# TheJacksonLaboratory/cnn_autoencoder

Measured on AMD Instinct MI355X. Metric: tiles/sec, compress+decompress round trip of 1024x1024x3 histology tiles, higher is better.
Workload: dtype f32 (f16x3 split MFMA: 3 f16 MFMAs per product, fp32 accumulate)

## Files before the change

### cnn_autoencoder_amd/_lib.py

```python
from __future__ import annotations

import ctypes
import os
import subprocess
import threading

import torch

_HERE = os.path.dirname(os.path.abspath(__file__))
LIB_PATH = os.environ.get('CAE_LIB') or os.path.join(_HERE, 'libcae_hip.so')
_lock = threading.Lock()
_lib = None

c_void_p = ctypes.c_void_p
c_int = ctypes.c_int
c_size_t = ctypes.c_size_t
c_float = ctypes.c_float

SYMBOLS = {
    'cae_version': (c_int, []),
    'cae_last_error': (ctypes.c_char_p, []),
    'cae_free': (None, [c_void_p]),
    'cae_model_create': (c_int, [c_int, c_int, c_int, c_int, c_int, ctypes.POINTER(c_void_p)]),
    'cae_model_destroy': (None, [c_void_p]),
    'cae_model_set_layer': (c_int, [c_void_p, c_int, c_int, c_int, c_int, c_void_p, c_void_p, c_void_p, c_void_p]),
    'cae_model_set_layer_act': (c_int, [c_void_p, c_int, c_int, c_int, c_void_p, c_void_p]),
    'cae_model_set_precision': (c_int, [c_void_p, c_int]),
    'cae_last_range_ticket': (ctypes.c_int64, []),
    'cae_range_check': (c_int, [c_void_p, ctypes.c_int64, c_void_p]),
    'cae_thread_force_fp32': (None, [c_int]),
    'cae_model_effective_precision': (c_int, [c_void_p, c_void_p]),
    'cae_model_set_entropy': (c_int, [c_void_p, c_int, c_int, c_void_p, c_void_p, c_void_p, c_void_p]),
    'cae_analysis': (c_int, [c_void_p, c_void_p, c_int, c_int, c_int, c_int, c_void_p, c_void_p]),
    'cae_analysis_levels': (c_int, [c_void_p, c_void_p, c_int, c_int, c_int, c_int, c_void_p, c_void_p, c_void_p]),
    'cae_synthesis': (c_int, [c_void_p, c_void_p, c_int, c_int, c_int, c_void_p, c_int, c_void_p, c_void_p]),
    'cae_model_set_layer_stage': (c_int, [c_void_p, c_int, c_int, c_int, c_void_p, c_void_p, c_void_p, c_void_p, c_int,
                                           c_int, c_int]),
    'cae_model_set_color_layer': (c_int, [c_void_p, c_int, c_int, c_int, c_void_p, c_void_p]),
    'cae_synthesis_multiscale': (c_int, [c_void_p, c_void_p, c_int, c_int, c_int, c_void_p, c_int, c_void_p, c_void_p,
                                          c_void_p]),
    'cae_analysis_symbols': (c_int, [c_void_p, c_void_p, c_int, c_int, c_int, c_int, c_void_p, c_void_p]),
    'cae_synthesis_symbols': (c_int, [c_void_p, c_void_p, c_int, c_int, c_int, c_void_p, c_int, c_void_p]),
    'cae_synthesis_scale': (c_int, [c_void_p, c_void_p, c_int, c_int, c_int, c_int, c_void_p, c_int, c_void_p]),
    'cae_synthesis_symbols_scale': (c_int, [c_void_p, c_void_p, c_int, c_int, c_int, c_int, c_void_p, c_int, c_void_p]),
    'cae_gdn_forward': (c_int, [c_void_p, c_int, c_int, c_void_p, c_int, c_int, c_int, c_void_p, c_void_p]),
    'cae_quantize': (c_int, [c_void_p, c_void_p, c_int, c_int, c_void_p, c_void_p]),
    'cae_quantize_export': (c_int, [c_void_p, c_void_p, c_int, c_int, c_void_p, c_int, c_void_p]),
    'cae_copy_to_host': (c_int, [c_void_p, c_void_p, c_size_t]),
    'cae_dequantize': (c_int, [c_void_p, c_void_p, c_int, c_int, c_void_p, c_void_p]),
    'cae_model_set_density': (c_int, [c_void_p, c_int, c_int, c_void_p, c_void_p, c_void_p, c_void_p, c_float]),
    'cae_model_set_likelihood_form': (c_int, [c_void_p, c_int]),
    'cae_likelihood': (c_int, [c_void_p, c_void_p, c_int, c_int, c_void_p, c_void_p, c_void_p, c_void_p]),
    'cae_tile_ssim': (c_int, [c_void_p, c_void_p, c_int, c_int, c_int, c_int, c_void_p, c_void_p, c_size_t, c_void_p]),
    'cae_tile_delta_e': (c_int, [c_void_p, c_void_p, c_int, c_size_t, c_void_p, c_void_p, c_size_t, c_void_p]),
    'cae_u8hwc_to_planes': (c_int, [c_void_p, c_int, c_int, c_int, c_int, c_void_p, c_void_p]),
    'cae_avgpool2': (c_int, [c_void_p, c_int, c_int, c_int, c_void_p, c_void_p]),
    'cae_msssim_level': (c_int, [c_void_p, c_void_p, c_int, c_int, c_int, c_void_p, c_void_p, c_void_p, c_size_t, c_void_p]),
    'cae_tile_sse': (c_int, [c_void_p, c_void_p, c_int, c_size_t, c_void_p, c_void_p]),
    'cae_model_set_profiling': (c_int, [c_void_p, c_int]),
    'cae_model_get_profile': (c_int, [c_void_p, c_int, c_void_p, c_int, c_void_p, c_int]),
    'cae_t_packed_bytes': (c_size_t, [c_int, c_int, c_int]),
    'cae_t_pack_weights': (c_int, [c_void_p, c_int, c_int, c_int, c_int, c_void_p, c_void_p]),
    'cae_t_from_nchw': (c_int, [c_void_p, c_int, c_int, c_int, c_int, c_int, c_void_p, c_void_p, c_void_p]),
    'cae_t_to_nchw': (c_int, [c_void_p, c_int, c_int, c_int, c_int, c_int, c_void_p, c_void_p]),
    'cae_t_set_samples_per_block': (c_int, [c_int]),
# ... 220 lines not shown
```

### cnn_autoencoder_amd/csrc/cae_api.hip

```cpp
#include "cae_hip.h"
#include "cae_internal.hpp"
#include "cae_kernels.hpp"
#include "cae_kernels_f16.hpp"
#include "cae_launch.hpp"
#include "cae_pack.hpp"

#include <algorithm>
#include <cmath>
#include <cstdio>
#include <cstdlib>
#include <cstring>
#include <string>

namespace cae {

thread_local std::string g_last_error;
thread_local int64_t g_last_ticket = 0;
thread_local int g_force_fp32 = 0;

int fail(int code, const char *fmt, ...) {
    char buf[512];
    va_list ap;
    va_start(ap, fmt);
    vsnprintf(buf, sizeof buf, fmt, ap);
// ... 5 lines not shown
void dev_free(void *p) { (void)hipFree(p); }

int DevBuf::alloc(size_t n) {
    reset();
    HIP_TRY(hipMalloc(&p, n));
    bytes = n;
    return CAE_OK;
}

int DevBuf::upload(const void *src, size_t n) {
    CAE_TRY(alloc(n));
    HIP_TRY(hipMemcpy(p, src, n, hipMemcpyHostToDevice));
    return CAE_OK;
}

int Model::ensure_ws(int which, size_t bytes) {
    DevBuf &b = ws[which];
    if (b.bytes >= bytes) return CAE_OK;
    if (b) {
        HIP_TRY(hipDeviceSynchronize());
        b.reset();
    }
    return b.alloc((bytes + (1u << 20)) & ~(size_t)((1u << 20) - 1));
}

int Model::order_stream(void *stream) {
    if (last_stream_set && last_stream != stream) {
        if (!order_event) HIP_TRY(hipEventCreateWithFlags((hipEvent_t *)&order_event, hipEventDisableTiming));
        HIP_TRY(hipEventRecord((hipEvent_t)order_event, (hipStream_t)last_stream));
        HIP_TRY(hipStreamWaitEvent((hipStream_t)stream, (hipEvent_t)order_event, 0));
    }
    last_stream = stream;
    last_stream_set = true;
    return CAE_OK;
}

int Model::ensure_device() {
    if (!zero) {
        CAE_TRY(zero.alloc(1024));
        HIP_TRY(hipMemset(zero.p, 0, 1024));
    }
    if (medians_dirty && ent.channels > 0) {
        CAE_TRY(medians_dev.upload(ent.medians));
        medians_dirty = false;
    }
    if (density_dirty && !density.empty()) {
// ... 570 lines not shown
            if ((rc = launch_conv(m->ks, l.ct, l.gdn, l.cin, a, st))) return rc;
        }
        prof.end();
        if (!last && levels && levels[i]) {
            const size_t t2 = (size_t)n * l.cout * a.OH * a.OW;
            if (f16)
                hipLaunchKernelGGL(c8s_to_nchw_kernel<false>, dim3(ew_grid(t2)), dim3(256), 0, st, (const char *)a.out,
                                   levels[i], n, l.cout, a.OH, a.OW, l.ct * 4);
            else
                hipLaunchKernelGGL(c8_to_nchw_kernel, dim3(ew_grid(t2)), dim3(256), 0, st, (const float *)a.out,
                                   levels[i], n, l.cout, a.OH * a.OW, l.ct * 4);
            HIP_TRY(hipGetLastError());
        }
        cur = (const float *)a.out;
        cur_planes = l.ct * 4;
        ch = a.OH;
        cw = a.OW;
        cur_idx = out_idx;
    }
    return CAE_OK;
}

static int synthesis_impl(cae_model_t *mm, const float *latents, const int32_t *symbols, int n, int lh, int lw, void *out,
                          int fmt, float *const *bridges, float *const *colors, void *stream, int scale = 0);

int cae_synthesis(cae_model_t *mm, const float *latents, int n, int lh, int lw, void *out, int fmt,
                  float *const *bridges, void *stream) {
    if (!latents) return fail(CAE_ERR_ARG, "NULL argument");
    return synthesis_impl(mm, latents, nullptr, n, lh, lw, out, fmt, bridges, nullptr, stream);
}

int cae_synthesis_multiscale(cae_model_t *mm, const float *latents, int n, int lh, int lw, void *out, int fmt,
                             float *const *bridges, float *const *colors, void *stream) {
    if (!latents) return fail(CAE_ERR_ARG, "NULL argument");
    return synthesis_impl(mm, latents, nullptr, n, lh, lw, out, fmt, bridges, colors, stream);
}

int cae_synthesis_symbols(cae_model_t *mm, const int32_t *symbols, int n, int lh, int lw, void *out, int fmt,
                          void *stream) {
    if (!symbols) return fail(CAE_ERR_ARG, "NULL argument");
    return synthesis_impl(mm, nullptr, symbols, n, lh, lw, out, fmt, nullptr, nullptr, stream);
}

static int check_scale(cae_model_t *mm, int scale) {
    Model *m = reinterpret_cast<Model *>(mm);
    if (!m) return fail(CAE_ERR_ARG, "NULL argument");
    if (scale < 0 || scale >= m->L) return fail(CAE_ERR_ARG, "scale %d outside 0..%d", scale, m->L - 1);
    return CAE_OK;
}

int cae_synthesis_scale(cae_model_t *mm, const float *latents, int n, int lh, int lw, int scale, void *out, int fmt,
                        void *stream) {
    if (!latents) return fail(CAE_ERR_ARG, "NULL argument");
    CAE_TRY(check_scale(mm, scale));
    return synthesis_impl(mm, latents, nullptr, n, lh, lw, out, fmt, nullptr, nullptr, stream, scale);
}

int cae_synthesis_symbols_scale(cae_model_t *mm, const int32_t *symbols, int n, int lh, int lw, int scale, void *out,
                                int fmt, void *stream) {
    if (!symbols) return fail(CAE_ERR_ARG, "NULL argument");
    CAE_TRY(check_scale(mm, scale));
    return synthesis_impl(mm, nullptr, symbols, n, lh, lw, out, fmt, nullptr, nullptr, stream, scale);
}

static int synthesis_impl(cae_model_t *mm, const float *latents, const int32_t *symbols, int n, int lh, int lw, void *out,
                          int fmt, float *const *bridges, float *const *colors, void *stream, int scale) {
    Model *m = reinterpret_cast<Model *>(mm);
    if (!m || !out) return fail(CAE_ERR_ARG, "NULL argument");
    const int stop = m->L - 1 - scale, nrun = stop + 1;
    if (symbols && m->ent.channels == 0) return fail(CAE_ERR_ARG, "entropy model not set");
    if (n < 1 || lh < 1 || lw < 1) return fail(CAE_ERR_ARG, "bad latent batch %dx%dx%d", n, lh, lw);
    if (fmt != CAE_FMT_U8_HWC && fmt != CAE_FMT_F32_NCHW) return fail(CAE_ERR_ARG, "bad pixel format %d", fmt);
    for (auto &l : m->dec)
        if (!l.set) return fail(CAE_ERR_ARG, "synthesis layer not set");
    for (int i = 0; colors && i + 1 < m->L; ++i)
        if (colors[i] && ((lh << (i + 1)) <= m->ks / 2 || (lw << (i + 1)) <= m->ks / 2))
            return fail(CAE_ERR_ARG, "colour layer %d input %d x %d too small for reflect padding %d", i, lh << (i + 1),
                        lw << (i + 1), m->ks / 2);
    if (scale > 0) {
        const Layer &l = m->dec[stop];
        if (!l.color_wp) return fail(CAE_ERR_ARG, "colour layer %d not set", stop);
        if ((lh << nrun) <= m->ks / 2 || (lw << nrun) <= m->ks / 2)
            return fail(CAE_ERR_ARG, "colour layer %d input %d x %d too small for reflect padding %d", stop, lh << nrun,
                        lw << nrun, m->ks / 2);
    }
    hipStream_t st = (hipStream_t)stream;
    std::lock_guard<std::mutex> lk(m->mu);
    int rc;
    if ((rc = m->ensure_device()) || (rc = m->order_stream(stream))) return rc;
// ... 28 lines not shown
    if (maxact && ((rc = m->ensure_ws(1, maxact)) || (rc = m->ensure_ws(2, maxact)))) return rc;
    if (maxact && need_third_slot && (rc = m->ensure_ws(3, maxact))) return rc;

    ProfScope prof(m, CAE_SYNTHESIS, st);
    prof.begin();
    const size_t tot = (size_t)n * p0 * lh * lw;
    if (f16)
        hipLaunchKernelGGL(nchw_to_c8s_kernel<true>, dim3(ew_grid(tot)), dim3(256), 0, st, latents, (char *)m->ws[0].p, n,
                           m->c_bn, lh, lw, p0, flag, symbols, m->medians_dev.get<float>());
    else
        hipLaunchKernelGGL(nchw_to_c8_kernel, dim3(ew_grid(tot)), dim3(256), 0, st, latents, (float *)m->ws[0].p, n,
                           m->c_bn, lh * lw, p0, symbols, m->medians_dev.get<float>());
    HIP_TRY(hipGetLastError());
    prof.end();

    bool use_pmap = false;
    if (f16 && scale == 0 && m->L >= 2 && m->ks == 3 && getenv("CAE_NO_PMAP") == nullptr) {
        const Layer &lp = m->dec[m->L - 2], &ll = m->dec[m->L - 1];
        use_pmap = ll.wp_pmap16 && !ll.gdn && ll.stages.empty() && lp.stages.empty() && lp.ct <= 4 && lp.cout == ll.cin &&
                   !(bridges && bridges[m->L - 2]) && !(colors && colors[m->L - 2]);
    }
    if (use_pmap) maxact = std::max(maxact, (size_t)n * (lh << (m->L - 1)) * (lw << (m->L - 1)) * 128);
    if (use_pmap && ((rc = m->ensure_ws(1, maxact)) || (rc = m->ensure_ws(2, maxact)))) return rc;

    const float *cur = (const float *)m->ws[0].p;
    int cur_planes = p0, ch = lh, cw = lw;
    int cur_idx = 0;
    for (int i = 0; i < nrun; ++i) {
        const Layer &l = m->dec[i];
        const bool last = i == m->L - 1;
        if (use_pmap && last) {
            prof.begin();
            const int gtx = (cw + 15) / 16, gty = (ch + 15) / 16;
            hipLaunchKernelGGL(pmap_gather_kernel, dim3((unsigned)((size_t)n * gtx * gty)), dim3(256), 0, st, cur,
                               l.bias.get<float>(), out, n, ch, cw, l.cout, fmt == CAE_FMT_U8_HWC ? OUT_U8HWC : OUT_NCHW, gtx,
                               gty);
            HIP_TRY(hipGetLastError());
            prof.end();
            break;
        }
        if (!l.stages.empty() && (rc = run_stages(m, l, true, n, ch, cw, cur, cur_idx, cur_planes, st, f16, flag))) return rc;
        const int out_idx = pick_slot(cur_idx, cur_idx);
        LayerArgs a = layer_args(m, cur, cur_planes, last ? out : m->ws[out_idx].p, n, ch, cw, 2 * ch, 2 * cw, l.ct, l.cout,
                                 last ? (fmt == CAE_FMT_U8_HWC ? OUT_U8HWC : OUT_NCHW) : OUT_C8, l.act, flag);
        a.wp = l.wp.get<float>();
        a.bias = l.bias.get<float>();
        a.gp = l.gp.get<float>();
        a.beta = l.beta.get<float>();
        if (use_pmap && i == m->L - 2) {
            a.outfmt = OUT_PMAP;
            a.pm = m->dec[m->L - 1].wp_pmap16.p;
        }
        prof.begin();
        if (f16) {
            a.gp = l.gp16.get<float>();
            if (last && l.wp_edge16 && last_f16_fits(m->ks, l.cin)) {
                a.wp = l.wp_edge16.get<float>();
                if ((rc = launch_last_f16(m->ks, l.cin, a, st))) return rc;
            } else {
                if (l.act && l.ct > 4)
// ... 26 lines not shown
            HIP_TRY(hipGetLastError());
        }
        cur = (const float *)a.out;
        cur_planes = l.ct * 4;
        ch = a.OH;
        cw = a.OW;
        cur_idx = out_idx;
    }
    if (scale > 0) {
        const Layer &l = m->dec[stop];
        const int ofmt = fmt == CAE_FMT_U8_HWC ? OUT_U8HWC : OUT_NCHW;
        prof.begin();
        if (l.color_w4) {
            if ((rc = launch_color_small(m->ks, f16, cur, cur_planes, l.cout, l.color_w4.get<float>(),
                                         l.color_bias.get<float>(), n, ch, cw, l.color_cout, out, ofmt, flag, st)))
                return rc;
        } else {
            float *img = ofmt == OUT_NCHW ? (float *)out : (float *)m->ws[pick_slot(cur_idx, cur_idx)].p;
            if ((rc = launch_color(m, l, f16, cur, cur_planes, n, ch, cw, img, flag, st))) return rc;
            if (ofmt == OUT_U8HWC && (rc = launch_nchw_to_u8hwc(img, out, n, l.color_cout, (size_t)ch * cw, st))) return rc;
        }
        prof.end();
    }
    return CAE_OK;
}

int cae_gdn_forward(cae_model_t *mm, int track, int index, const float *x, int n, int h, int w, float *y, void *stream) {
    Model *m = reinterpret_cast<Model *>(mm);
    if (!m || !x || !y) return fail(CAE_ERR_ARG, "NULL argument");
    Layer *lp;
    CAE_TRY(layer_of(m, track, index, lp));
    if (n < 1 || h < 1 || w < 1) return fail(CAE_ERR_ARG, "bad tensor shape");
    hipStream_t st = (hipStream_t)stream;
    std::lock_guard<std::mutex> lk(m->mu);
    const Layer &l = *lp;
    if (!l.set || !l.gdn) return fail(CAE_ERR_ARG, "layer has no GDN");
    const int planes = l.ct * 4;
    int rc;
    if ((rc = m->ensure_device()) || (rc = m->order_stream(stream))) return rc;
    if ((rc = m->ensure_ws(0, (size_t)n * planes * h * w * 32))) return rc;
    const size_t tot = (size_t)n * planes * h * w;
    hipLaunchKernelGGL(nchw_to_c8_kernel, dim3(ew_grid(tot)), dim3(256), 0, st, x, (float *)m->ws[0].p, n, l.cout, h * w,
                       planes);
    HIP_TRY(hipGetLastError());
    LayerArgs a = layer_args(m, (const float *)m->ws[0].p, planes, y, n, h, w, h, w, l.ct, l.cout, OUT_NCHW, 0, nullptr);
    a.gp = l.gp.get<float>();
// ... 285 lines not shown
```

### cnn_autoencoder_amd/csrc/cae_internal.hpp

```cpp
#pragma once
#include <cstdarg>
#include <cstddef>
#include <cstdint>
#include <mutex>
#include <utility>
#include <vector>

namespace cae {

int fail(int code, const char *fmt, ...);

void dev_free(void *p);

struct DevBuf {
    void *p = nullptr;
    size_t bytes = 0;
    DevBuf() = default;
    DevBuf(DevBuf &&o) noexcept : p(o.p), bytes(o.bytes) {
        o.p = nullptr;
        o.bytes = 0;
    }
    DevBuf &operator=(DevBuf &&o) noexcept {
        if (this != &o) {
            reset();
// ... 80 lines not shown
    DevBuf buf;
    uint64_t version = 0;
    size_t enc = 0, cdf = 0, lut = 0, len = 0, off = 0;
};

struct Model {
    int c_org = 0, c_net = 0, c_bn = 0, L = 0, ks = 3;
    std::vector<Layer> enc, dec;
    EntropyTables ent;
    uint64_t ent_version = 0;
    DevEntropy ent_dev;
    int ensure_ent_device();
    DevBuf medians_dev;
    bool medians_dirty = false;
    std::vector<float> density;
    int density_r = 0, density_k = 0, density_per_channel = 0;
    float density_bound = 0.f;
    int likelihood_plain = 1;
    DevBuf density_dev;
    bool density_dirty = false;
    DevBuf bits_ws;
    DevBuf zero;
    DevBuf ws[4];
    std::mutex mu;
    int precision = 0;
    bool profiling = false;
    std::vector<std::vector<std::pair<void *, void *>>> prof[2];
    static constexpr int kFlagSlots = 1024;
    int *flags = nullptr;
    int *flags_dev = nullptr;
    int64_t flag_seq = 0;
    int *next_flag(int64_t *ticket);
    bool f16_usable() const;
    int ensure_ws(int which, size_t bytes);
    int ensure_device();
    void *last_stream = nullptr;
    bool last_stream_set = false;
    void *order_event = nullptr;
    int order_stream(void *stream);
    ~Model();
};

}
```

### cnn_autoencoder_amd/csrc/cae_kernels_f16.hpp

```cpp
#pragma once
#include "cae_kernels.hpp"

namespace cae {

constexpr int F16_ISSUERS = 2;
#define ISSUER(w, NW, NI) ((w) < (NI) ? (w) : -1)

typedef _Float16 f16x8 __attribute__((ext_vector_type(8)));
typedef _Float16 f16x4 __attribute__((ext_vector_type(4)));


__device__ __forceinline__ void split_f16(float v, _Float16 &hi, _Float16 &lo) {
    hi = (_Float16)v;
    lo = (_Float16)(v - (float)hi);
}

typedef unsigned u32x2v __attribute__((ext_vector_type(2)));
__device__ __forceinline__ u32x2v split2_f16(float a, float b) {
    typedef float f32x2 __attribute__((ext_vector_type(2)));
    typedef _Float16 f16x2 __attribute__((ext_vector_type(2)));
    const f32x2 ab = {a, b};
    const unsigned hi = __builtin_bit_cast(unsigned, __builtin_convertvector(ab, f16x2));
    float l0, l1;
    asm("v_fma_mix_f32 %0, %1, -1.0, %2 op_sel_hi:[1,0,0]" : "=v"(l0) : "v"(hi), "v"(a));
// ... 735 lines not shown
            const f16x8 ah = *(const f16x8 *)(ab + ((jt * 2 + s) * 2 + 0) * 1024);
            const f16x8 al = *(const f16x8 *)(ab + ((jt * 2 + s) * 2 + 1) * 1024);
            pm = mfma3(ah, al, sh, sl, pm);
        }
    raise_if_over(mx, p.flag);
    __builtin_amdgcn_wave_barrier();
#pragma unroll
    for (int g = 0; g < 4; ++g) {
        const f32x4 v = {pm[4 * g], pm[4 * g + 1], pm[4 * g + 2], pm[4 * g + 3]};
        *(f32x4 *)(tbuf + m * 128 + (((2 * g + h) ^ (m & 7)) * 16)) = v;
    }
    __builtin_amdgcn_wave_barrier();
    const int half_w = p.OW >> 1, j0u = __builtin_amdgcn_readfirstlane(j0);
    float *rec0 = (float *)p.out + ((((size_t)n * p.OH + oy) * 2 + par) * half_w + j0u) * 32 + 4 * lane;
#pragma unroll
    for (int it = 0; it < 4; ++it) {
        const int px = (lane >> 3) + 8 * it, q = lane & 7;
        const f32x4 v = *(const f32x4 *)(tbuf + px * 128 + ((q ^ (px & 7)) * 16));
        if (row_valid && j0u + px < half_w) *(f32x4 *)(rec0 + it * 256) = v;
    }
    __builtin_amdgcn_wave_barrier();
}

static __global__ void __launch_bounds__(256) pmap_gather_kernel(const float *pm, const float *bias, void *out, int N, int H,
                                                               int W, int cout, int fmt, int tiles_x, int tiles_y) {
    constexpr int T = 16, R = T + 1, PITCH = 36;
    __shared__ __attribute__((aligned(16))) float rec[R * R * PITCH];
    __shared__ __attribute__((aligned(4))) uint8_t orow[2 * T][2 * T * 3 + 4];
    int bid = blockIdx.x;
    const int tx = bid % tiles_x;
    bid /= tiles_x;
    const int ty = bid % tiles_y;
    const int n = bid / tiles_y;
    const int a0 = ty * T, b0 = tx * T;
    constexpr int NIT = (R * R * 8 + 255) / 256;
    f32x4 stage[NIT];
#pragma unroll
    for (int it = 0; it < NIT; ++it) {
        const int i = threadIdx.x + it * 256;
        const int q = i & 7, r = i >> 3;
        const int ra = r / R, rb = r - ra * R;
        const int a = a0 + ra, b = b0 + rb;
        stage[it] = f32x4{0.0f, 0.0f, 0.0f, 0.0f};
        if (i < R * R * 8 && a < H && b < W) stage[it] = *(const f32x4 *)(pm + pmap_record(n, H, W, a, b) + 4 * q);
    }
#pragma unroll
    for (int it = 0; it < NIT; ++it) {
        const int i = threadIdx.x + it * 256;
        if (i < R * R * 8) *(f32x4 *)(rec + (i >> 3) * PITCH + 4 * (i & 7)) = stage[it];
    }
    __syncthreads();
    const int la = threadIdx.x >> 4, lb = threadIdx.x & 15;
    const int a = a0 + la, b = b0 + lb;
    const float *p00 = rec + (la * R + lb) * PITCH, *p01 = p00 + PITCH, *p10 = p00 + R * PITCH, *p11 = p10 + PITCH;
    const int OH = 2 * H, OW = 2 * W;
    const bool u8 = fmt == OUT_U8HWC;
    typedef float f32x2 __attribute__((ext_vector_type(2)));
    const f32x4 s0 = *(const f32x4 *)(p00), s1 = *(const f32x4 *)(p00 + 4), s2 = *(const f32x4 *)(p00 + 8);
    const f32x4 l0 = *(const f32x4 *)(p01 + 12), u0 = *(const f32x4 *)(p10 + 20), d0 = *(const f32x4 *)(p11 + 28);
    const f32x2 l1 = *(const f32x2 *)(p01 + 16), u1 = *(const f32x2 *)(p10 + 24);
    const float self[12] = {s0[0], s0[1], s0[2], s0[3], s1[0], s1[1], s1[2], s1[3], s2[0], s2[1], s2[2], s2[3]};
    const float left[6] = {l0[0], l0[1], l0[2], l0[3], l1[0], l1[1]};
    const float up[6] = {u0[0], u0[1], u0[2], u0[3], u1[0], u1[1]};
    const float diag[3] = {d0[0], d0[1], d0[2]};
#pragma unroll
    for (int c = 0; c < 3; ++c) {
        if (c >= cout) break;
        const float bs = bias ? bias[c] : 0.0f;
        const float o00 = bs + self[c];
        const float o01 = bs + self[3 + c] + left[c];
        const float o10 = bs + self[6 + c] + up[c];
        const float o11 = bs + self[9 + c] + left[3 + c] + up[3 + c] + diag[c];
        if (u8) {
            orow[2 * la][(2 * lb) * cout + c] = clip_u8(o00 * 255.0f);
            orow[2 * la][(2 * lb + 1) * cout + c] = clip_u8(o01 * 255.0f);
            orow[2 * la + 1][(2 * lb) * cout + c] = clip_u8(o10 * 255.0f);
            orow[2 * la + 1][(2 * lb + 1) * cout + c] = clip_u8(o11 * 255.0f);
        } else if (a < H && b < W) {
            float *o = (float *)out + (((size_t)n * cout + c) * OH + 2 * a) * OW + 2 * b;
            o[0] = o00;
            o[1] = o01;
            o[OW] = o10;
            o[OW + 1] = o11;
        }
    }
    if (!u8) return;
    __syncthreads();
    const int row_bytes = 2 * T * cout;
    const int valid_rows = min(2 * T, OH - 2 * a0), valid_bytes = min(2 * T, OW - 2 * b0) * cout;
    uint8_t *obase = (uint8_t *)out + (((size_t)n * OH + 2 * a0) * OW + 2 * b0) * cout;
    const bool dwords = ((((size_t)OW * cout) & 3) == 0) && (((uintptr_t)obase & 3) == 0) && (row_bytes & 3) == 0 &&
                        valid_bytes == row_bytes;
    if (dwords) {
        const int per_row = row_bytes / 4;
        for (int i = threadIdx.x; i < valid_rows * per_row; i += 256) {
            const int r = i / per_row, q = i - r * per_row;
            *(uint32_t *)(obase + (size_t)r * OW * cout + 4 * q) = *(const uint32_t *)(&orow[r][4 * q]);
        }
    } else {
        for (int i = threadIdx.x; i < valid_rows * valid_bytes; i += 256) {
            const int r = i / valid_bytes, q = i - r * valid_bytes;
            obase[(size_t)r * OW * cout + q] = orow[r][q];
        }
    }
}

template <int KS, int CT, int NW, int PT, bool IGDN>
struct DeconvGeomF16 {
    static constexpr int P = KS / 2;
    static constexpr int DLO = -((P + 1) / 2), DHI = (KS - 1 - P) / 2;
    static constexpr int WH = 32 + DHI - DLO;
    static constexpr int ROWS = NW * PT;
    static constexpr int NSTRAY = WH - 32;
    static constexpr int AL_INSTR = 4 * ROWS * 32 / 64;
    static constexpr int AL_BYTES = AL_INSTR * 1024;
    static constexpr int STRAY_INSTR = (NSTRAY * 4 * ROWS + 63) / 64;
    static constexpr int HALO_INSTR = AL_INSTR + STRAY_INSTR;
    static_assert((4 * ROWS * 32) % 64 == 0 && 64 % (4 * ROWS) == 0, "halo image assumes 4, 8 or 16 input rows per block");
    static constexpr int W_INSTR = KS * CT * 2;
    static constexpr int W_BYTES = W_INSTR * 1024;
    static constexpr int G_BYTES = IGDN ? CT * 4096 : 0;
    static constexpr int CONV_STAGE = W_BYTES + HALO_INSTR * 1024;
    static constexpr int STAGE_BYTES = CONV_STAGE > G_BYTES ? CONV_STAGE : G_BYTES;
    static constexpr int NI = NW / F16_ISSUERS > 0 ? NW / F16_ISSUERS : 1;
    static constexpr int MAXP = (HALO_INSTR + NI - 1) / NI;
    static constexpr int AL_PER = AL_INSTR / NI, AL_STEP = NI * 64 / (ROWS * 32);
    static_assert(AL_INSTR % NI == 0 && (NI * 64) % (ROWS * 32) == 0 && AL_STEP <= 2 && STRAY_INSTR <= NI,
// ... 438 lines not shown
```

### cnn_autoencoder_amd/modules.py

```python
from __future__ import annotations

import ctypes
import math
from typing import List, Optional, Tuple

import numpy as np
import torch
import torch.nn as nn

from . import _lib
from .entropy import LowerBound

REPARAM_OFFSET = 2.0 ** -18


class RangeTicket:

    def __init__(self, track, handle, ticket: int, call):
        self._track, self._handle, self.ticket, self._call = track, handle, int(ticket), call

    def overflowed(self) -> bool:
        if self.ticket == 0:
            return False
        over = ctypes.c_int(0)
# ... 621 lines not shown
                                   dtype=torch.float32, device=dev) for i, u in enumerate(self._units()[:-1])]
                brg_ptr = (ctypes.c_void_p * (L - 1))(*[b.data_ptr() for b in brg])
            col: List[torch.Tensor] = []
            col_ptr = None
            if colors and self.multiscale_analysis and L > 1:
                col = [torch.empty((n, self._dims[0], lh * 2 ** (i + 1), lw * 2 ** (i + 1)), dtype=torch.float32,
                                   device=dev) for i in range(L - 1)]
                col_ptr = (ctypes.c_void_p * (L - 1))(*[c.data_ptr() for c in col])
            _lib.check(_lib.lib().cae_synthesis_multiscale(hd.ptr, x.data_ptr(), n, lh, lw, out.data_ptr(), fmt,
                                                           brg_ptr, col_ptr, _lib.stream_ptr()))
            return out, brg, col
        return self._guarded(hd, call)

    def forward(self, x: torch.Tensor, bridges: bool = True):
        from . import train
        if train.needs_grad(self, x):
            if x.dim() != 4 or x.size(1) != self._dims[2]:
                raise ValueError(f'expected (B,{self._dims[2]},h,w), got {tuple(x.shape)}')
            return train.synthesis_forward(self, x)
        out, brg, col = self._run(x, _lib.FMT_F32_NCHW, bridges, colors=True)
        x_r = [out] + (col[::-1] if col else [None] * (self._dims[3] - 1))
        return x_r, brg + [out]

    def forward_u8(self, x: torch.Tensor) -> torch.Tensor:
        out, _, _ = self._run(x, _lib.FMT_U8_HWC, False)
        return out

    def _check_scale(self, scale) -> int:
        L = self._dims[3]
        if isinstance(scale, bool) or int(scale) != scale:
            raise ValueError(f'scale must be an integer, got {scale!r}')
        scale = int(scale)
        if not 0 <= scale < L:
            raise ValueError(f'scale {scale} outside 0..{L - 1}')
        if scale > 0 and not self.multiscale_analysis:
            raise ValueError('scale > 0 needs a model built with multiscale_analysis=True (colour layers)')
        return scale

    def _run_scale(self, x: torch.Tensor, scale: int, fmt: int):
        scale = self._check_scale(scale)
        dev = _lib.require_gpu()
        if x.dim() != 4 or x.size(1) != self._dims[2]:
            raise ValueError(f'expected (B,{self._dims[2]},h,w), got {tuple(x.shape)}')
        hd = self._sync()
        x = x.detach().to(device=dev, dtype=torch.float32).contiguous()
        n, _, lh, lw = x.shape
        up = 2 ** (self._dims[3] - scale)

        def call():
            if fmt == _lib.FMT_U8_HWC:
                out = torch.empty((n, lh * up, lw * up, self._dims[0]), dtype=torch.uint8, device=dev)
            else:
                out = torch.empty((n, self._dims[0], lh * up, lw * up), dtype=torch.float32, device=dev)
            _lib.check(_lib.lib().cae_synthesis_scale(hd.ptr, x.data_ptr(), n, lh, lw, scale, out.data_ptr(), fmt,
                                                      _lib.stream_ptr()))
            return out
        return self._guarded(hd, call)

    def forward_scale(self, x: torch.Tensor, scale: int) -> torch.Tensor:
        return self._run_scale(x, scale, _lib.FMT_F32_NCHW)

    def forward_scale_u8(self, x: torch.Tensor, scale: int) -> torch.Tensor:
        return self._run_scale(x, scale, _lib.FMT_U8_HWC)

    def forward_symbols_u8(self, sym: torch.Tensor, eb, defer: bool = False, scale: int = 0):
        scale = self._check_scale(scale)
        dev = _lib.require_gpu()
        if sym.dim() != 4 or sym.size(1) != self._dims[2] or sym.dtype != torch.int32:
            raise ValueError(f'expected int32 (B,{self._dims[2]},h,w), got {sym.dtype} {tuple(sym.shape)}')
        if eb.channels != self._dims[2]:
            raise ValueError(f'entropy model has {eb.channels} channels, the latents {self._dims[2]}')
        sym = sym.to(dev).contiguous()
        hd = self._sync_entropy(eb)
        n, _, lh, lw = sym.shape
        L = self._dims[3]

        def call():
            up = 2 ** (L - scale)
            out = torch.empty((n, lh * up, lw * up, self._dims[0]), dtype=torch.uint8, device=dev)
            if scale == 0:
                _lib.check(_lib.lib().cae_synthesis_symbols(hd.ptr, sym.data_ptr(), n, lh, lw, out.data_ptr(),
                                                            _lib.FMT_U8_HWC, _lib.stream_ptr()))
            else:
                _lib.check(_lib.lib().cae_synthesis_symbols_scale(hd.ptr, sym.data_ptr(), n, lh, lw, scale,
                                                                  out.data_ptr(), _lib.FMT_U8_HWC, _lib.stream_ptr()))
            return out
        return self._guarded(hd, call, defer)
```

### cnn_autoencoder_amd/slide.py

```python
from __future__ import annotations

import math
import time
from typing import Dict, List, Sequence, Tuple

import numpy as np
import torch

STATS_WIDTH = 3


def tile_range(rank: int, world: int, n_tiles: int) -> Tuple[int, int]:
    if not (0 <= rank < world) or n_tiles < 0:
        raise ValueError(f'bad partition request rank={rank} world={world} n_tiles={n_tiles}')
    base, rem = divmod(n_tiles, world)
    lo = rank * base + min(rank, rem)
    hi = lo + base + (1 if rank < rem else 0)
    return lo, hi


def tile_stats(nbytes: Sequence[int], sse: Sequence[float], n_samples: int) -> torch.Tensor:
    out = torch.empty((len(nbytes), STATS_WIDTH), dtype=torch.float64)
    out[:, 0] = torch.tensor(list(nbytes), dtype=torch.float64)
    out[:, 1] = torch.tensor(list(sse), dtype=torch.float64)
# ... 139 lines not shown
        return self.eb.encode_symbols(sym_host, self.coder_threads)

    @torch.no_grad()
    def decompress(self, payloads: Sequence[bytes], h: int, w: int, scale: int = 0) -> torch.Tensor:
        scale = self.dec._check_scale(scale)
        size = (h // 2 ** self.level, w // 2 ** self.level)
        y_q = self.eb.decompress(payloads, size, coder=self.coder)
        return self.dec.forward_scale_u8(y_q, scale) if scale else self.dec.forward_u8(y_q)

    @torch.no_grad()
    def tile_sse(self, rec: torch.Tensor, tiles: torch.Tensor) -> torch.Tensor:
        from . import _lib
        n = tiles.shape[0]
        rec, tiles = rec.contiguous(), tiles.contiguous()
        out = torch.empty(n, dtype=torch.float64, device=tiles.device)
        _lib.check(_lib.lib().cae_tile_sse(rec.data_ptr(), tiles.data_ptr(), n, tiles[0].numel(), out.data_ptr(),
                                           _lib.stream_ptr()))
        return out

    @torch.no_grad()
    def roundtrip(self, tiles_dev: torch.Tensor) -> Tuple[List[bytes], torch.Tensor, torch.Tensor]:
        n, h, w, c = tiles_dev.shape
        payloads = self.compress(tiles_dev)
        rec = self.decompress(payloads, h, w)
        sse = self.tile_sse(rec, tiles_dev).cpu()
        stats = tile_stats([len(p) + 16 for p in payloads], sse.tolist(), h * w * c)
        return payloads, rec, stats

    def _ring(self, name: str) -> _PinnedRing:
        d = self.depth
        slots = {
            't': 2,
            'a': d + 1,
            'd': d + 2,
            'o': 4,
            's': 3,
            'c': 4,
        }[name]
        ring = self._rings.get(name)
        if ring is None or ring.slots != slots:
            ring = self._rings[name] = _PinnedRing(slots)
        return ring

    def _h2d_stream(self):
        if self._copy_stream is None:
            self._copy_stream = torch.cuda.Stream(_dev())
        return self._copy_stream

# ... 44 lines not shown
            payloads = self.eb.encode_symbols_device(sym)
        _clock(tm, 'host_encode', t0)
        return payloads

    def _encode_async(self, k, t, main, pull_pool, enc_pool, packed, tm=None):
        sym, guard, ready, pin = self._launch_analysis(k, t, main)
        if self.coder == 'device':
            return enc_pool.submit(self._device_encode, k, sym, guard, ready, main, tm)
        pulled = pull_pool.submit(self._pull, sym, guard, ready, pin, main, tm)
        return enc_pool.submit(self._host_encode, pulled, packed, tm)

    def _decode(self, k, payloads, hw, tm=None):
        t0 = time.perf_counter()
        if self.coder == 'device':
            stream = self._coder_stream(k)
            with torch.cuda.device(stream.device), torch.cuda.stream(stream):
                sym = self.eb.decode_symbols_device(payloads, hw)
        else:
            sym = self._ring('d').take(k, (len(payloads), self.eb.channels, hw), torch.int32)
            self.eb.decode_symbols(payloads, hw, self.decode_threads, out=sym.numpy())
        _clock(tm, 'host_decode', t0)
        return sym

    def _launch_synthesis(self, k, sym, lh, lw, main, up, scale=0):
        if self.coder != 'device':
            with torch.cuda.stream(up):
                sym = sym.to(main.device, non_blocking=True)
                copied = torch.cuda.Event(blocking=True)
                copied.record(up)
            self._ring('d').read_by(k, copied)
            main.wait_event(copied)
        sym.record_stream(main)
        return self.dec.forward_symbols_u8(sym.reshape(sym.size(0), self.eb.channels, lh, lw), self.eb, defer=True,
                                           scale=scale)

    def _to_device(self, batch, k, up, main):
        if isinstance(batch, torch.Tensor) and batch.is_cuda:
            return batch
        arr = batch.numpy() if isinstance(batch, torch.Tensor) else np.ascontiguousarray(batch)
        if arr.dtype != np.uint8 or arr.ndim != 4:
            raise ValueError(f'expected a (n,h,w,c) uint8 batch, got {arr.dtype} {arr.shape}')
        pin = self._ring('t').take(k, arr.shape, torch.uint8)
        pin.numpy()[...] = arr
        with torch.cuda.stream(up):
            dev = pin.to(_dev(), non_blocking=True)
            copied = torch.cuda.Event(blocking=True)
            copied.record(up)
        self._ring('t').read_by(k, copied)
        main.wait_event(copied)
        dev.record_stream(main)
        return dev

    @torch.no_grad()
    def compress_batches(self, batches):
        from concurrent.futures import ThreadPoolExecutor
        main = torch.cuda.current_stream(_dev())
        up = self._h2d_stream()
# ... 55 lines not shown
    @torch.no_grad()
    def run(self, batches: Sequence[torch.Tensor], keep_payloads: bool = False):
        from concurrent.futures import ThreadPoolExecutor
        main = torch.cuda.current_stream(batches[0].device)
        copy_up = self._h2d_stream()
        K = len(batches)
        DEPTH = self.depth
        tm = {key: [] for key in ('host_encode', 'host_decode', 'wait_host', 'd2h_copy')}
        all_payloads, stats_parts = [], []
        device = self.coder == 'device'
        n0, h0, w0, _ = batches[0].shape
        lh0, lw0 = self.enc.latent_size(h0, w0)
        for ring in ([] if device else [self._ring('a'), self._ring('d')]):
            for j in range(ring.slots):
                ring.take(j, (n0, self.eb.channels, lh0 * lw0), torch.int32)

        def decode(k, encoded, hw):
            payloads = encoded.result()
            return payloads, self._decode(k, payloads, hw, tm)

        def stage_d(k, payloads, sym):
            t = batches[k]
            n, h, w, c = t.shape
            rec, guard = self._launch_synthesis(k, sym, h // 2 ** self.level, w // 2 ** self.level, main, copy_up)
            sse = self.tile_sse(rec, t)
            got = torch.cuda.Event()
            got.record(main)
            sse_host = self._ring('s').take(k, (n,), torch.float64)
            with torch.cuda.stream(copy_up):
                copy_up.wait_event(got)
                sse_host.copy_(sse, non_blocking=True)
                landed = torch.cuda.Event(blocking=True)
                landed.record(copy_up)
            sse.record_stream(copy_up)
            nbytes = ([payloads.nbytes(i) + 16 for i in range(len(payloads))] if hasattr(payloads, 'nbytes')
                      else [len(p) + 16 for p in payloads])
            return k, sse_host, landed, guard, nbytes, h * w * c

        pending = []

        def finalize(k, sse_pinned, landed, guard, nbytes, samples):
            rec = self._in_range(None, guard, landed, main)
            sse_host = sse_pinned.tolist()
            if rec is not None:
                sse_host = self.tile_sse(rec, batches[k]).cpu().tolist()
            stats_parts.append(tile_stats(nbytes, sse_host, samples))

        workers = DEPTH if device else 1
        with ThreadPoolExecutor(max_workers=1) as pull_pool, ThreadPoolExecutor(max_workers=workers) as enc_pool, \
                ThreadPoolExecutor(max_workers=workers) as dec_pool:
            futs = {}

            def submit(k):
                lh, lw = self.enc.latent_size(*batches[k].shape[1:3])
                encoded = self._encode_async(k, batches[k], main, pull_pool, enc_pool, not keep_payloads, tm)
                futs[k] = dec_pool.submit(decode, k, encoded, lh * lw)

            for k in range(min(DEPTH, K)):
                submit(k)
            for k in range(K):
                if k + DEPTH < K:
                    submit(k + DEPTH)
                t0 = time.perf_counter()
                payloads, sym = futs.pop(k).result()
                _clock(tm, 'wait_host', t0)
                pending.append(stage_d(k, payloads, sym))
                if keep_payloads:
                    all_payloads.append(payloads)
# ... 141 lines not shown
```

### include/cae_hip.h

```cpp
#ifndef CAE_HIP_H
#define CAE_HIP_H

#include <stddef.h>
#include <stdint.h>

#ifdef __cplusplus
extern "C" {
#endif

typedef struct cae_model cae_model_t;

enum cae_status {
    CAE_OK = 0,
    CAE_ERR_ARG = -1,
    CAE_ERR_HIP = -2,
    CAE_ERR_NOMEM = -3,
    CAE_ERR_UNSUPPORTED = -4,
    CAE_ERR_CORRUPT = -5,
    CAE_ERR_RANGE = -6
};

enum cae_track { CAE_ANALYSIS = 0, CAE_SYNTHESIS = 1 };
enum cae_pixfmt {
    CAE_FMT_U8_HWC = 0,
// ... 25 lines not shown
                          const int32_t *cdf_length_host, const int32_t *offset_host,
                          const float *medians_host);

int cae_analysis(cae_model_t *m, const void *tiles_dev, int fmt, int n, int h, int w,
                 float *latents_dev, void *stream);

int cae_analysis_levels(cae_model_t *m, const void *tiles_dev, int fmt, int n, int h, int w, float *latents_dev,
                        float *const *levels_dev, void *stream);

int cae_synthesis(cae_model_t *m, const float *latents_dev, int n, int lh, int lw,
                  void *out_dev, int fmt, float *const *bridges_dev, void *stream);

int cae_model_set_layer_stage(cae_model_t *m, int track, int index, int stage, const float *w, const float *bias,
                              const float *beta, const float *gamma, int act, int add_residual, int post_act);

int cae_model_set_color_layer(cae_model_t *m, int index, int cin, int cout, const float *w, const float *bias);
int cae_synthesis_multiscale(cae_model_t *m, const float *latents_dev, int n, int lh, int lw, void *out_dev, int fmt,
                             float *const *bridges_dev, float *const *colors_dev, void *stream);

int cae_analysis_symbols(cae_model_t *m, const void *tiles_dev, int fmt, int n, int h, int w, int32_t *symbols_dev,
                         void *stream);
int cae_synthesis_symbols(cae_model_t *m, const int32_t *symbols_dev, int n, int lh, int lw, void *out_dev, int fmt,
                          void *stream);

int cae_synthesis_scale(cae_model_t *m, const float *latents_dev, int n, int lh, int lw, int scale, void *out_dev,
                        int fmt, void *stream);
int cae_synthesis_symbols_scale(cae_model_t *m, const int32_t *symbols_dev, int n, int lh, int lw, int scale,
                                void *out_dev, int fmt, void *stream);

int cae_gdn_forward(cae_model_t *m, int track, int index, const float *x_dev, int n, int h, int w,
                    float *y_dev, void *stream);

int cae_quantize(cae_model_t *m, const float *latents_dev, int n, int hw, int32_t *symbols_dev, void *stream);
int cae_dequantize(cae_model_t *m, const int32_t *symbols_dev, int n, int hw, float *latents_dev, void *stream);

int cae_quantize_export(cae_model_t *m, const float *latents_dev, int n, int hw, int32_t *symbols_pinned_host,
                        int max_blocks, void *stream);

int cae_model_set_density(cae_model_t *m, int channels, int n_filters, const int *filters,
                          const float *const *matrices, const float *const *biases,
                          const float *const *factors, float likelihood_bound);

int cae_model_set_likelihood_form(cae_model_t *m, int form);

int cae_likelihood(cae_model_t *m, const float *latents_dev, int n, int hw, float *y_hat_dev,
                   float *likelihood_dev, double *bits_dev, void *stream);
// ... 255 lines not shown
```

Before: 4179.

## Fuse per-tile SSE against originals into final pmap gather kernel

Adds a synthesis entry point that computes per-tile squared error against the original uint8 tiles inside the last pixel-map gather kernel. The original bytes are loaded alongside the output, squared differences are computed with udot4, and partial sums are reduced through sharded 64-bit atomics and a small finish kernel. This removes the separate tile_sse pass that re-read the reconstructed and original tiles. It also skips global loads of record fields the halo row or column never uses. The round-trip and pipelined paths now call the fused variant, at the cost of extra registers in the gather kernel and an extra tiny launch.

```diff
diff --git a/cnn_autoencoder_amd/_lib.py b/cnn_autoencoder_amd/_lib.py
--- a/cnn_autoencoder_amd/_lib.py
+++ b/cnn_autoencoder_amd/_lib.py
@@ -41,6 +41,8 @@
                                           c_void_p]),
     'cae_analysis_symbols': (c_int, [c_void_p, c_void_p, c_int, c_int, c_int, c_int, c_void_p, c_void_p]),
     'cae_synthesis_symbols': (c_int, [c_void_p, c_void_p, c_int, c_int, c_int, c_void_p, c_int, c_void_p]),
+    'cae_synthesis_u8_sse': (c_int, [c_void_p, c_void_p, c_void_p, c_int, c_int, c_int, c_void_p, c_void_p, c_void_p,
+                                      c_void_p]),
     'cae_synthesis_scale': (c_int, [c_void_p, c_void_p, c_int, c_int, c_int, c_int, c_void_p, c_int, c_void_p]),
     'cae_synthesis_symbols_scale': (c_int, [c_void_p, c_void_p, c_int, c_int, c_int, c_int, c_void_p, c_int, c_void_p]),
     'cae_gdn_forward': (c_int, [c_void_p, c_int, c_int, c_void_p, c_int, c_int, c_int, c_void_p, c_void_p]),
diff --git a/cnn_autoencoder_amd/csrc/cae_api.hip b/cnn_autoencoder_amd/csrc/cae_api.hip
--- a/cnn_autoencoder_amd/csrc/cae_api.hip
+++ b/cnn_autoencoder_amd/csrc/cae_api.hip
@@ -51,6 +51,21 @@
         b.reset();
     }
     return b.alloc((bytes + (1u << 20)) & ~(size_t)((1u << 20) - 1));
+}
+
+int Model::ensure_sse_acc(int n) {
+    const int npad = (n + 15) / 16 * 16;
+    if (sse_acc && sse_npad >= npad) return CAE_OK;
+    if (sse_acc) {
+        HIP_TRY(hipDeviceSynchronize());
+        sse_acc.reset();
+    }
+    const size_t bytes = (size_t)PMAP_SSE_SHARDS * npad * sizeof(unsigned long long);
+    CAE_TRY(sse_acc.alloc(bytes));
+    HIP_TRY(hipMemset(sse_acc.p, 0, bytes));
+    HIP_TRY(hipDeviceSynchronize());
+    sse_npad = npad;
+    return CAE_OK;
 }
 
 int Model::order_stream(void *stream) {
@@ -667,7 +682,8 @@
 }
 
 static int synthesis_impl(cae_model_t *mm, const float *latents, const int32_t *symbols, int n, int lh, int lw, void *out,
-                          int fmt, float *const *bridges, float *const *colors, void *stream, int scale = 0);
+                          int fmt, float *const *bridges, float *const *colors, void *stream, int scale = 0,
+                          const uint8_t *original = nullptr, double *sse = nullptr);
 
 int cae_synthesis(cae_model_t *mm, const float *latents, int n, int lh, int lw, void *out, int fmt,
                   float *const *bridges, void *stream) {
@@ -685,6 +701,14 @@
                           void *stream) {
     if (!symbols) return fail(CAE_ERR_ARG, "NULL argument");
     return synthesis_impl(mm, nullptr, symbols, n, lh, lw, out, fmt, nullptr, nullptr, stream);
+}
+
+int cae_synthesis_u8_sse(cae_model_t *mm, const float *latents, const int32_t *symbols, int n, int lh, int lw, uint8_t *out,
+                         const uint8_t *original, double *sse, void *stream) {
+    if (!latents == !symbols) return fail(CAE_ERR_ARG, "exactly one of latents and symbols");
+    if (!original != !sse) return fail(CAE_ERR_ARG, "original tiles and sse go together");
+    if (sse && n > 65535) return fail(CAE_ERR_ARG, "bad shape");
+    return synthesis_impl(mm, latents, symbols, n, lh, lw, out, CAE_FMT_U8_HWC, nullptr, nullptr, stream, 0, original, sse);
 }
 
 static int check_scale(cae_model_t *mm, int scale) {
@@ -709,7 +733,8 @@
 }
 
 static int synthesis_impl(cae_model_t *mm, const float *latents, const int32_t *symbols, int n, int lh, int lw, void *out,
-                          int fmt, float *const *bridges, float *const *colors, void *stream, int scale) {
+                          int fmt, float *const *bridges, float *const *colors, void *stream, int scale,
+                          const uint8_t *original, double *sse) {
     Model *m = reinterpret_cast<Model *>(mm);
     if (!m || !out) return fail(CAE_ERR_ARG, "NULL argument");
     const int stop = m->L - 1 - scale, nrun = stop + 1;
@@ -784,6 +809,8 @@
     }
     if (use_pmap) maxact = std::max(maxact, (size_t)n * (lh << (m->L - 1)) * (lw << (m->L - 1)) * 128);
     if (use_pmap && ((rc = m->ensure_ws(1, maxact)) || (rc = m->ensure_ws(2, maxact)))) return rc;
+    const bool sse_in_gather = sse && use_pmap;
+    if (sse_in_gather && (rc = m->ensure_sse_acc(n))) return rc;
 
     const float *cur = (const float *)m->ws[0].p;
     int cur_planes = p0, ch = lh, cw = lw;
@@ -796,8 +823,13 @@
             const int gtx = (cw + 15) / 16, gty = (ch + 15) / 16;
             hipLaunchKernelGGL(pmap_gather_kernel, dim3((unsigned)((size_t)n * gtx * gty)), dim3(256), 0, st, cur,
                                l.bias.get<float>(), out, n, ch, cw, l.cout, fmt == CAE_FMT_U8_HWC ? OUT_U8HWC : OUT_NCHW, gtx,
-                               gty);
+                               gty, sse_in_gather ? original : nullptr, m->sse_acc.get<unsigned long long>(), m->sse_npad);
             HIP_TRY(hipGetLastError());
+            if (sse_in_gather) {
+                hipLaunchKernelGGL(pmap_sse_finish_kernel, dim3((n * PMAP_SSE_SHARDS + 255) / 256), dim3(256), 0, st,
+                                   m->sse_acc.get<unsigned long long>(), m->sse_npad, n, sse);
+                HIP_TRY(hipGetLastError());
+            }
             prof.end();
             break;
         }
@@ -870,6 +902,9 @@
         }
         prof.end();
     }
+    if (sse && !sse_in_gather)
+        return cae_tile_sse((const uint8_t *)out, original, n, (size_t)(lh << m->L) * (lw << m->L) * m->dec[m->L - 1].cout,
+                            sse, stream);
     return CAE_OK;
 }
 
diff --git a/cnn_autoencoder_amd/csrc/cae_internal.hpp b/cnn_autoencoder_amd/csrc/cae_internal.hpp
--- a/cnn_autoencoder_amd/csrc/cae_internal.hpp
+++ b/cnn_autoencoder_amd/csrc/cae_internal.hpp
@@ -126,6 +126,9 @@
     DevBuf bits_ws;
     DevBuf zero;
     DevBuf ws[4];
+    DevBuf sse_acc;
+    int sse_npad = 0;
+    int ensure_sse_acc(int n);
     std::mutex mu;
     int precision = 0;
     bool profiling = false;
diff --git a/cnn_autoencoder_amd/csrc/cae_kernels_f16.hpp b/cnn_autoencoder_amd/csrc/cae_kernels_f16.hpp
--- a/cnn_autoencoder_amd/csrc/cae_kernels_f16.hpp
+++ b/cnn_autoencoder_amd/csrc/cae_kernels_f16.hpp
@@ -781,39 +781,65 @@
     __builtin_amdgcn_wave_barrier();
 }
 
+constexpr int PMAP_SSE_SHARDS = 16;
 static __global__ void __launch_bounds__(256) pmap_gather_kernel(const float *pm, const float *bias, void *out, int N, int H,
-                                                               int W, int cout, int fmt, int tiles_x, int tiles_y) {
+                                                               int W, int cout, int fmt, int tiles_x, int tiles_y,
+                                                               const uint8_t *orig, unsigned long long *acc, int npad) {
     constexpr int T = 16, R = T + 1, PITCH = 36;
     __shared__ __attribute__((aligned(16))) float rec[R * R * PITCH];
     __shared__ __attribute__((aligned(4))) uint8_t orow[2 * T][2 * T * 3 + 4];
+    __shared__ unsigned wave_part[4];
     int bid = blockIdx.x;
     const int tx = bid % tiles_x;
     bid /= tiles_x;
     const int ty = bid % tiles_y;
     const int n = bid / tiles_y;
     const int a0 = ty * T, b0 = tx * T;
+    const int OH = 2 * H, OW = 2 * W;
+    const bool u8 = fmt == OUT_U8HWC;
+    const int row_bytes = 2 * T * cout, per_row = row_bytes / 4;
+    const int valid_rows = min(2 * T, OH - 2 * a0), valid_bytes = min(2 * T, OW - 2 * b0) * cout;
+    const size_t obase_off = (((size_t)n * OH + 2 * a0) * OW + 2 * b0) * cout, opitch = (size_t)OW * cout;
+    uint8_t *obase = (uint8_t *)out + obase_off;
+    const bool dwords = ((opitch & 3) == 0) && (((uintptr_t)obase & 3) == 0) && (row_bytes & 3) == 0 &&
+                        valid_bytes == row_bytes;
+    constexpr int NDW = 2 * T * 2 * T * 3 / 4 / 256;
+    const uint8_t *gbase = orig ? orig + obase_off : nullptr;
+    const bool gdwords = u8 && gbase && dwords && ((uintptr_t)gbase & 3) == 0;
+    uint32_t gdw[NDW] = {};
+    if (gdwords) {
+#pragma unroll
+        for (int k = 0; k < NDW; ++k) {
+            const int i = min((int)threadIdx.x + k * 256, valid_rows * per_row - 1);
+            const int r = i / per_row, q = i - r * per_row;
+            gdw[k] = *(const uint32_t *)(gbase + r * opitch + 4 * q);
+        }
+    }
     constexpr int NIT = (R * R * 8 + 255) / 256;
     f32x4 stage[NIT];
+    unsigned loaded = 0;
 #pragma unroll
     for (int it = 0; it < NIT; ++it) {
         const int i = threadIdx.x + it * 256;
         const int q = i & 7, r = i >> 3;
         const int ra = r / R, rb = r - ra * R;
         const int a = a0 + ra, b = b0 + rb;
-        stage[it] = f32x4{0.0f, 0.0f, 0.0f, 0.0f};
-        if (i < R * R * 8 && a < H && b < W) stage[it] = *(const f32x4 *)(pm + pmap_record(n, H, W, a, b) + 4 * q);
+        const bool col = rb == T, row = ra == T;
+        const bool used = !(col || row) || q == 7 || (col && !row && (q == 3 || q == 4)) || (row && !col && (q == 5 || q == 6));
+        const bool ok = i < R * R * 8 && a < H && b < W && used;
+        loaded |= (unsigned)ok << it;
+        stage[it] = *(const f32x4 *)(ok ? pm + pmap_record(n, H, W, a, b) + 4 * q : pm);
     }
 #pragma unroll
     for (int it = 0; it < NIT; ++it) {
         const int i = threadIdx.x + it * 256;
-        if (i < R * R * 8) *(f32x4 *)(rec + (i >> 3) * PITCH + 4 * (i & 7)) = stage[it];
+        if (i < R * R * 8)
+            *(f32x4 *)(rec + (i >> 3) * PITCH + 4 * (i & 7)) = (loaded >> it) & 1 ? stage[it] : f32x4{0.0f, 0.0f, 0.0f, 0.0f};
     }
     __syncthreads();
     const int la = threadIdx.x >> 4, lb = threadIdx.x & 15;
     const int a = a0 + la, b = b0 + lb;
     const float *p00 = rec + (la * R + lb) * PITCH, *p01 = p00 + PITCH, *p10 = p00 + R * PITCH, *p11 = p10 + PITCH;
-    const int OH = 2 * H, OW = 2 * W;
-    const bool u8 = fmt == OUT_U8HWC;
     typedef float f32x2 __attribute__((ext_vector_type(2)));
     const f32x4 s0 = *(const f32x4 *)(p00), s1 = *(const f32x4 *)(p00 + 4), s2 = *(const f32x4 *)(p00 + 8);
     const f32x4 l0 = *(const f32x4 *)(p01 + 12), u0 = *(const f32x4 *)(p10 + 20), d0 = *(const f32x4 *)(p11 + 28);
@@ -845,23 +871,50 @@
     }
     if (!u8) return;
     __syncthreads();
-    const int row_bytes = 2 * T * cout;
-    const int valid_rows = min(2 * T, OH - 2 * a0), valid_bytes = min(2 * T, OW - 2 * b0) * cout;
-    uint8_t *obase = (uint8_t *)out + (((size_t)n * OH + 2 * a0) * OW + 2 * b0) * cout;
-    const bool dwords = ((((size_t)OW * cout) & 3) == 0) && (((uintptr_t)obase & 3) == 0) && (row_bytes & 3) == 0 &&
-                        valid_bytes == row_bytes;
+    unsigned part = 0;
     if (dwords) {
-        const int per_row = row_bytes / 4;
-        for (int i = threadIdx.x; i < valid_rows * per_row; i += 256) {
+#pragma unroll
+        for (int k = 0; k < NDW; ++k) {
+            const int i = threadIdx.x + k * 256;
+            if (i >= valid_rows * per_row) break;
             const int r = i / per_row, q = i - r * per_row;
-            *(uint32_t *)(obase + (size_t)r * OW * cout + 4 * q) = *(const uint32_t *)(&orow[r][4 * q]);
+            const uint32_t v = *(const uint32_t *)(&orow[r][4 * q]);
+            *(uint32_t *)(obase + r * opitch + 4 * q) = v;
+            if (gdwords)
+                part += __builtin_amdgcn_udot4(v, v, __builtin_amdgcn_udot4(gdw[k], gdw[k], 0u, false), false) -
+                        2u * __builtin_amdgcn_udot4(v, gdw[k], 0u, false);
         }
     } else {
         for (int i = threadIdx.x; i < valid_rows * valid_bytes; i += 256) {
             const int r = i / valid_bytes, q = i - r * valid_bytes;
-            obase[(size_t)r * OW * cout + q] = orow[r][q];
-        }
-    }
+            obase[r * opitch + q] = orow[r][q];
+        }
+    }
+    if (!gbase) return;
+    if (!gdwords)
+        for (int i = threadIdx.x; i < valid_rows * valid_bytes; i += 256) {
+            const int r = i / valid_bytes, q = i - r * valid_bytes;
+            const int d = (int)orow[r][q] - (int)gbase[r * opitch + q];
+            part += (unsigned)(d * d);
+        }
+#pragma unroll
+    for (int off = 32; off > 0; off >>= 1) part += __shfl_down(part, off, 64);
+    if ((threadIdx.x & 63) == 0) wave_part[threadIdx.x >> 6] = part;
+    __syncthreads();
+    if (threadIdx.x == 0) {
+        const int s = (ty * tiles_x + tx) % PMAP_SSE_SHARDS;
+        const unsigned long long sum = (unsigned long long)wave_part[0] + wave_part[1] + wave_part[2] + wave_part[3];
+        __hip_atomic_fetch_add(acc + (size_t)s * npad + n, sum, __ATOMIC_RELAXED, __HIP_MEMORY_SCOPE_AGENT);
+    }
+}
+
+static __global__ void __launch_bounds__(256) pmap_sse_finish_kernel(unsigned long long *acc, int npad, int N, double *sse) {
+    const int i = blockIdx.x * 256 + threadIdx.x, tile = i / PMAP_SSE_SHARDS, s = i % PMAP_SSE_SHARDS;
+    unsigned long long v = 0;
+    if (tile < N) v = __hip_atomic_exchange(acc + (size_t)s * npad + tile, 0ull, __ATOMIC_RELAXED, __HIP_MEMORY_SCOPE_AGENT);
+#pragma unroll
+    for (int off = PMAP_SSE_SHARDS / 2; off > 0; off >>= 1) v += __shfl_xor(v, off, PMAP_SSE_SHARDS);
+    if (tile < N && s == 0) sse[tile] = (double)v;
 }
 
 template <int KS, int CT, int NW, int PT, bool IGDN>
diff --git a/cnn_autoencoder_amd/modules.py b/cnn_autoencoder_amd/modules.py
--- a/cnn_autoencoder_amd/modules.py
+++ b/cnn_autoencoder_amd/modules.py
@@ -667,9 +667,31 @@
         x_r = [out] + (col[::-1] if col else [None] * (self._dims[3] - 1))
         return x_r, brg + [out]
 
-    def forward_u8(self, x: torch.Tensor) -> torch.Tensor:
-        out, _, _ = self._run(x, _lib.FMT_U8_HWC, False)
-        return out
+    def _u8_sse(self, hd, latents, sym, n: int, lh: int, lw: int, original: torch.Tensor):
+        up = 2 ** self._dims[3]
+        shape = (n, lh * up, lw * up, self._dims[0])
+        if original.dtype != torch.uint8 or tuple(original.shape) != shape or not original.is_cuda:
+            raise ValueError(f'expected the original tiles as uint8 {shape} on the GPU, got {original.dtype} '
+                             f'{tuple(original.shape)} on {original.device}')
+        original = original.contiguous()
+        out = torch.empty(shape, dtype=torch.uint8, device=original.device)
+        sse = torch.empty(n, dtype=torch.float64, device=original.device)
+        _lib.check(_lib.lib().cae_synthesis_u8_sse(hd.ptr, None if latents is None else latents.data_ptr(),
+                                                   None if sym is None else sym.data_ptr(), n, lh, lw, out.data_ptr(),
+                                                   original.data_ptr(), sse.data_ptr(), _lib.stream_ptr()))
+        return out, sse
+
+    def forward_u8(self, x: torch.Tensor, original: Optional[torch.Tensor] = None):
+        if original is None:
+            out, _, _ = self._run(x, _lib.FMT_U8_HWC, False)
+            return out
+        dev = _lib.require_gpu()
+        hd = self._sync()
+        if x.dim() != 4 or x.size(1) != self._dims[2]:
+            raise ValueError(f'expected (B,{self._dims[2]},h,w), got {tuple(x.shape)}')
+        x = x.detach().to(device=dev, dtype=torch.float32).contiguous()
+        n, _, lh, lw = x.shape
+        return self._guarded(hd, lambda: self._u8_sse(hd, x, None, n, lh, lw, original))
 
     def _check_scale(self, scale) -> int:
         L = self._dims[3]
@@ -708,8 +730,11 @@
     def forward_scale_u8(self, x: torch.Tensor, scale: int) -> torch.Tensor:
         return self._run_scale(x, scale, _lib.FMT_U8_HWC)
 
-    def forward_symbols_u8(self, sym: torch.Tensor, eb, defer: bool = False, scale: int = 0):
+    def forward_symbols_u8(self, sym: torch.Tensor, eb, defer: bool = False, scale: int = 0,
+                           original: Optional[torch.Tensor] = None):
         scale = self._check_scale(scale)
+        if original is not None and scale:
+            raise ValueError('the squared error against the original tiles is formed at full resolution: scale 0')
         dev = _lib.require_gpu()
         if sym.dim() != 4 or sym.size(1) != self._dims[2] or sym.dtype != torch.int32:
             raise ValueError(f'expected int32 (B,{self._dims[2]},h,w), got {sym.dtype} {tuple(sym.shape)}')
@@ -721,6 +746,8 @@
         L = self._dims[3]
 
         def call():
+            if original is not None:
+                return self._u8_sse(hd, None, sym, n, lh, lw, original)
             up = 2 ** (L - scale)
             out = torch.empty((n, lh * up, lw * up, self._dims[0]), dtype=torch.uint8, device=dev)
             if scale == 0:
diff --git a/cnn_autoencoder_amd/slide.py b/cnn_autoencoder_amd/slide.py
--- a/cnn_autoencoder_amd/slide.py
+++ b/cnn_autoencoder_amd/slide.py
@@ -185,8 +185,9 @@
     def roundtrip(self, tiles_dev: torch.Tensor) -> Tuple[List[bytes], torch.Tensor, torch.Tensor]:
         n, h, w, c = tiles_dev.shape
         payloads = self.compress(tiles_dev)
-        rec = self.decompress(payloads, h, w)
-        sse = self.tile_sse(rec, tiles_dev).cpu()
+        y_q = self.eb.decompress(payloads, (h // 2 ** self.level, w // 2 ** self.level), coder=self.coder)
+        rec, sse = self.dec.forward_u8(y_q, original=tiles_dev)
+        sse = sse.cpu()
         stats = tile_stats([len(p) + 16 for p in payloads], sse.tolist(), h * w * c)
         return payloads, rec, stats
 
@@ -277,7 +278,7 @@
         _clock(tm, 'host_decode', t0)
         return sym
 
-    def _launch_synthesis(self, k, sym, lh, lw, main, up, scale=0):
+    def _launch_synthesis(self, k, sym, lh, lw, main, up, scale=0, original=None):
         if self.coder != 'device':
             with torch.cuda.stream(up):
                 sym = sym.to(main.device, non_blocking=True)
@@ -287,7 +288,7 @@
             main.wait_event(copied)
         sym.record_stream(main)
         return self.dec.forward_symbols_u8(sym.reshape(sym.size(0), self.eb.channels, lh, lw), self.eb, defer=True,
-                                           scale=scale)
+                                           scale=scale, original=original)
 
     def _to_device(self, batch, k, up, main):
         if isinstance(batch, torch.Tensor) and batch.is_cuda:
@@ -389,8 +390,8 @@
         def stage_d(k, payloads, sym):
             t = batches[k]
             n, h, w, c = t.shape
-            rec, guard = self._launch_synthesis(k, sym, h // 2 ** self.level, w // 2 ** self.level, main, copy_up)
-            sse = self.tile_sse(rec, t)
+            (rec, sse), guard = self._launch_synthesis(k, sym, h // 2 ** self.level, w // 2 ** self.level, main, copy_up,
+                                                       original=t)
             got = torch.cuda.Event()
             got.record(main)
             sse_host = self._ring('s').take(k, (n,), torch.float64)
@@ -407,10 +408,10 @@
         pending = []
 
         def finalize(k, sse_pinned, landed, guard, nbytes, samples):
-            rec = self._in_range(None, guard, landed, main)
+            again = self._in_range(None, guard, landed, main)
             sse_host = sse_pinned.tolist()
-            if rec is not None:
-                sse_host = self.tile_sse(rec, batches[k]).cpu().tolist()
+            if again is not None:
+                sse_host = again[1].cpu().tolist()
             stats_parts.append(tile_stats(nbytes, sse_host, samples))
 
         workers = DEPTH if device else 1
diff --git a/include/cae_hip.h b/include/cae_hip.h
--- a/include/cae_hip.h
+++ b/include/cae_hip.h
@@ -71,6 +71,9 @@
                          void *stream);
 int cae_synthesis_symbols(cae_model_t *m, const int32_t *symbols_dev, int n, int lh, int lw, void *out_dev, int fmt,
                           void *stream);
+
+int cae_synthesis_u8_sse(cae_model_t *m, const float *latents_dev, const int32_t *symbols_dev, int n, int lh, int lw,
+                         uint8_t *out_dev, const uint8_t *original_dev, double *sse_dev, void *stream);
 
 int cae_synthesis_scale(cae_model_t *m, const float *latents_dev, int n, int lh, int lw, int scale, void *out_dev,
                         int fmt, void *stream);
```

After: 4205, median of 4. No clear change (+0.6%).
